# huzi96/gaussian-pcloud-render

Measured on AMD Instinct MI355X. Metric: rendered frames/sec at 1080p (fwd+bwd), THuman-800K, higher is better.
Workload: dtype f32

## Files before the change

### gaussian-pcloud-render_amd/csrc/api.hip

```cpp
#include <algorithm>
#include <cstdarg>
#include <cstdio>
#include <cstring>
#include <string>
#include <vector>

#include "common.hpp"
#include <atomic>
#include <map>
#include <mutex>

namespace gsr {

static thread_local char g_err[512] = "";

static int fail(int code, const char* fmt, ...)
{
    va_list ap;
    va_start(ap, fmt);
    vsnprintf(g_err, sizeof(g_err), fmt, ap);
    va_end(ap);
    return code;
}

// ... 117 lines not shown
        return fail(GSR_ERR_INVALID, "[gsr] %lld tiles x %d views: too many for one launch", (long long)(gx * gy), V);
    return GSR_OK;
}

static int tile_bits(int T) { return (int)higher_msb((uint32_t)T); }
static int sorted_buffer(int T) { return ((tile_bits(T) + RADIX_BITS - 1) / RADIX_BITS) & 1; }

static inline void* align256(void* p) { return (void*)(((uintptr_t)p + 255) & ~(uintptr_t)255); }

static int make_batch(const gsr_params* p, int V, void* geom, size_t geom_bytes, void* image, size_t image_bytes, void* binning,
                      size_t binning_bytes, bool with_grad, Batch& B)
{
    B.V = V;
    const size_t G = geom_view(nullptr, p->P).bytes, I = image_view(nullptr, p->W, p->H).bytes;
    const size_t GR = with_grad ? grad_rec_bytes(p->P) : 0;
    if (!geom || geom_bytes < (size_t)V * (G + GR) + 256)
        return fail(GSR_ERR_CAPACITY, "[gsr] geom arena too small (%zu < %zu%s)", geom_bytes, (size_t)V * (G + GR) + 256,
                    with_grad ? ", need_backward" : "");
    if (!image || image_bytes < (size_t)V * I + 256)
        return fail(GSR_ERR_CAPACITY, "[gsr] image arena too small (%zu < %zu)", image_bytes, (size_t)V * I + 256);
    B.g = geom_view(align256(geom), p->P);
    B.g_stride = G;
    B.grad_rec = with_grad ? reinterpret_cast<float*>(reinterpret_cast<char*>(align256(geom)) + (size_t)V * G) : nullptr;
    B.gr_stride = GR;
    B.iv = image_view(align256(image), p->W, p->H);
    B.iv_stride = I;
    if (binning) {
        if (binning_bytes < 256 + 256 * (size_t)V) return fail(GSR_ERR_CAPACITY, "[gsr] binning arena too small");
        const size_t per_view = ((binning_bytes - 256) / (size_t)V) / 256 * 256;
        const int64_t cap = bin_capacity_from_bytes(per_view);
        if (cap < 1) return fail(GSR_ERR_CAPACITY, "[gsr] binning arena too small (%zu bytes for %d views)", binning_bytes, V);
        B.b = bin_view(align256(binning), cap > 0xFFFFFFFFll ? 0xFFFFFFFFll : cap);
        B.b_stride = per_view;
    } else {
        B.b = bin_view(nullptr, 1);
        B.b.cap = 0;
        B.b_stride = 0;
    }
    return GSR_OK;
}

struct FrameRecord {
    int kind = 0;
    int need_backward = 0;
    int nx = 0, layout = 0;
    int V = 0, P = 0, W = 0, H = 0;
// ... 382 lines not shown
        int64_t n = list_pairs >= 0 ? list_pairs : B.b.cap;
        if (n > B.b.cap) n = B.b.cap;
        if (n < 1) n = 1;
        const size_t need = gsr_backward_det_bytes(V, p->P, p->W, p->H, n);
        if (!det->scratch || det->bytes < need)
            return fail(GSR_ERR_CAPACITY, "[gsr] backward_det: scratch block too small (%zu < %zu = gsr_backward_det_bytes(%d, %d, %d, %d, %lld): "
                        "the forward's lists hold up to %lld pairs per view)", det->bytes, need, V, p->P, p->W, p->H, (long long)n,
                        (long long)n);
        D = det_view(align256(det->scratch), T, n);
        d_stride = det_view_bytes(p->W, p->H, n);
    }
    if (x) {
        const int nx = x->X.nx;
        x->X.state = xstate_view(align256(const_cast<void*>(x->state)), p->W, p->H, B.b.cap, nx);
        x->X.state_stride = xstate_view_bytes(p->W, p->H, B.b.cap, nx);
        if (x->state_bytes < (size_t)V * x->X.state_stride + 256)
            return fail(GSR_ERR_CAPACITY, "[gsr] extra-state block too small for this binning arena");
    }
    {
        ProfScope ps("bwd_items", L.stream);
        const size_t n_out = !x ? 0 : (size_t)p->P * (x->layout == 0 ? x->X.nx : x->layout == 1 ? V * x->X.nx : (1 + V) * 4);
        if (x && hipMemsetAsync(x->XG.grad, 0, n_out * sizeof(float), L.stream) != hipSuccess)
            return fail(GSR_ERR_HIP, "[gsr] memset failed: %s", hipGetErrorString(hipGetLastError()));
        if (int e = launch_bwd_items(L, B, T, p->P)) return e;
    }
    int dres = 0;
    if (det) {
        {
            ProfScope ps("det_prepare", L.stream);
            if (int e = launch_det_prepare(L, B, D, d_stride, B.b.val[res], T)) return e;
        }
        {
            ProfScope ps("det_sort", L.stream);
            if (int e = launch_det_sort(L, B, D, d_stride, p->P, &dres)) return e;
        }
    }
    {
        ProfScope ps("render_backward", L.stream);
        const RenderBwdDet d{D.part, D.flags, D.slot_base, d_stride, (uint32_t)D.cap};
        if (int e = launch_render_backward(L, *p, B, B.b.val[res], G.dL_dpix, x ? &x->X : nullptr, x ? &x->XG : nullptr, det ? &d : nullptr))
            return e;
    }
    if (det) {
        ProfScope ps("det_reduce", L.stream);
        if (int e = launch_det_reduce(L, B, D, d_stride, dres)) return e;
    }
    {
// ... 279 lines not shown
```

### gaussian-pcloud-render_amd/csrc/binning.hip

```cpp
#include "common.hpp"
#include "tile_cull.hpp"

namespace gsr {

__device__ __forceinline__ uint64_t agent_load(const uint64_t* p)
{
    return __hip_atomic_load(p, __ATOMIC_RELAXED, __HIP_MEMORY_SCOPE_AGENT);
}
__device__ __forceinline__ void agent_store(uint64_t* p, uint64_t v)
{
    __hip_atomic_store(p, v, __ATOMIC_RELAXED, __HIP_MEMORY_SCOPE_AGENT);
}

#ifdef GSR_STATS
constexpr int DUP_REC = 65536;
__device__ unsigned g_dup_rec[DUP_REC][4];
#define DUP_T(var) const unsigned long long var = wall_clock64()
#define DUP_ADD(i, v) do { if (threadIdx.x == 0) { const unsigned r_ = blockIdx.y * gridDim.x + s_ticket; if (r_ < DUP_REC) g_dup_rec[r_][i] = (unsigned)(v); } } while (0)
int debug_dup_times(unsigned long long* out8, int reset)
{
    static unsigned host[DUP_REC][4];
    if (hipMemcpyFromSymbol(host, HIP_SYMBOL(g_dup_rec), sizeof(host)) != hipSuccess) return -1;
    for (int i = 0; i < 8; i++) out8[i] = 0;
    for (int r = 0; r < DUP_REC; r++) {
// ... 398 lines not shown
                cur[2 * lane + 1] = inc - a1;
            }
            __syncthreads();
        }
    }
}

static void order_params(float& knee, float& expo)
{
    static const float k = [] { const char* e = getenv("GSR_ORDER_KNEE"); return e ? (float)atof(e) : 2048.f; }();
    static const float x = [] { const char* e = getenv("GSR_ORDER_EXP"); return e ? (float)atof(e) : 0.3f; }();
    knee = k;
    expo = x;
}

int launch_tile_order(const Launch& L, const Batch& B, int T)
{
    float knee, expo;
    order_params(knee, expo);
    hipLaunchKernelGGL(k_tile_order, dim3(B.V), dim3(1024), 0, L.stream, T, B.iv.ranges, B.iv.tile_order, B.iv_stride, knee, expo);
    return check_launch(L, "tile_order");
}

constexpr int BWD_CLEAR_BLOCKS = 64;
__global__ __launch_bounds__(1024) void k_bwd_items(int T, int chunk_shift, const uint32_t* __restrict__ need, uint32_t* __restrict__ items,
                                                    uint32_t* __restrict__ count, size_t iv_stride, const uint64_t* __restrict__ counters,
                                                    size_t g_stride, float* __restrict__ grad_rec, size_t gr_stride, size_t gr_bytes)
{
    if (blockIdx.y != 0) {
        if (at_view(counters, g_stride, blockIdx.x)[CNT_BWD_DIRTY] == 0) return;
        zero_region(reinterpret_cast<char*>(at_view(grad_rec, gr_stride, blockIdx.x)), gr_bytes,
                    (size_t)(blockIdx.y - 1) * 1024 + threadIdx.x, (size_t)BWD_CLEAR_BLOCKS * 1024);
        return;
    }
    need = at_view(need, iv_stride, blockIdx.x);
    items = at_view(items, iv_stride, blockIdx.x);
    count = at_view(count, iv_stride, blockIdx.x);
    if (threadIdx.x < 8) count[BWD_QUEUE_WORD + threadIdx.x] = 0;
    __shared__ uint32_t cnt[ORD_BUCKETS];
    __shared__ uint32_t cur[ORD_BUCKETS];
    const uint32_t lane = threadIdx.x & 63;
    if (threadIdx.x < ORD_BUCKETS) cnt[threadIdx.x] = 0;
    __syncthreads();
    const uint32_t full_bucket = work_bucket(1u << chunk_shift);
    for (int pass = 0; pass < 2; pass++) {
        for (int t = threadIdx.x; t < T; t += 1024) {
            const uint32_t n = need[t];
            if (n == 0) continue;
            uint32_t n_full = n >> chunk_shift;
            if (n_full > BWD_MAX_CHUNKS - 1) n_full = BWD_MAX_CHUNKS - 1;
            const uint32_t rest = n - (n_full << chunk_shift);
            if (pass == 0) {
                if (n_full) atomicAdd(&cnt[full_bucket], n_full);
                if (rest) atomicAdd(&cnt[work_bucket(rest)], 1u);
            } else {
                if (n_full) {
                    const uint32_t slot = atomicAdd(&cur[full_bucket], n_full);
// ... 1 lines not shown
                }
                if (rest) items[atomicAdd(&cur[work_bucket(rest)], 1u)] = (uint32_t)t | (n_full << BWD_TILE_BITS);
            }
        }
        __syncthreads();
        if (pass == 0) {
            if (threadIdx.x < 64) {
                const uint32_t a0 = cnt[2 * lane], a1 = cnt[2 * lane + 1];
                uint32_t inc = a0 + a1;
#pragma unroll
                for (int d = 1; d < 64; d <<= 1) {
                    const uint32_t n = __shfl_up(inc, d, 64);
                    if (lane >= (uint32_t)d) inc += n;
                }
                cur[2 * lane] = inc - a0 - a1;
                cur[2 * lane + 1] = inc - a1;
                if (lane == 63) count[0] = inc;
            }
            __syncthreads();
        }
    }
}

int launch_bwd_items(const Launch& L, const Batch& B, int T, int P)
{
    hipLaunchKernelGGL(k_bwd_items, dim3(B.V, 1 + BWD_CLEAR_BLOCKS), dim3(1024), 0, L.stream, T, B.chunk_shift(), B.iv.tile_need, B.iv.bwd_items,
                       B.iv.bwd_count, B.iv_stride, B.g.counters, B.g_stride, B.grad_rec, B.gr_stride, grad_rec_bytes(P));
    return check_launch(L, "bwd_items");
}

}
```

### gaussian-pcloud-render_amd/csrc/common.hpp

```cpp
#pragma once
#include <hip/hip_runtime.h>
#include <stdint.h>

#include <type_traits>

#include "../../include/gsr.h"

#if defined(__HIP_DEVICE_COMPILE__) && !defined(__gfx950__)
#error "libgsr_hip is written for gfx950 (MI355X) only: build with --offload-arch=gfx950"
#endif

namespace gsr {

constexpr int TILE_X = 16;
constexpr int TILE_Y = 16;
constexpr int TILE_PIX = TILE_X * TILE_Y;

constexpr int RS_THREADS = 256;
constexpr int RS_WAVES = RS_THREADS / 64;
#ifndef GSR_RS_ITEMS
#define GSR_RS_ITEMS 16
#endif
constexpr int RS_ITEMS = GSR_RS_ITEMS;
constexpr int RS_TILE = RS_THREADS * RS_ITEMS;
// ... 10 lines not shown
#endif
constexpr int DUP_G = GSR_DUP_G;
constexpr int DUP_BLOCK = DUP_THREADS * DUP_G;
#ifndef GSR_DUP_COPIES
#define GSR_DUP_COPIES 8
#endif
constexpr int DUP_COPIES = GSR_DUP_COPIES;

inline size_t align_up(size_t v, size_t a) { return (v + a - 1) / a * a; }
inline int64_t div_up(int64_t a, int64_t b) { return (a + b - 1) / b; }

template <typename T>
__host__ __device__ __forceinline__ T* at_view(T* p, size_t stride_bytes, uint32_t view)
{
    using B = typename std::conditional<std::is_const<T>::value, const char, char>::type;
    return (T*)((B*)p + stride_bytes * view);
}

struct __attribute__((aligned(64))) Splat {
    float4 q0, q1, q2, q3;
};

constexpr int GRAD_REC_WORDS = 16;
inline size_t grad_rec_bytes(int P) { return ((size_t)(P > 0 ? P : 1) * GRAD_REC_WORDS * sizeof(float) + 255) / 256 * 256; }

constexpr int CNT_NUM_RENDERED = 0;
constexpr int CNT_TRAP = 1;
constexpr int CNT_STALL = 2;
constexpr int CNT_NUM_REFERENCE = 4;
constexpr int LAND_NUM_REFERENCE = 3;
constexpr int CNT_BWD_DIRTY = 3;

struct GeomView {
    Splat* splat;
    uint32_t* tiles_touched;
    uint8_t* clamped;
    uint32_t* dkey[2];
    uint32_t* dval[2];
    uint32_t* hist;
    uint32_t* totals;
    uint32_t* blk_minmax;
    uint32_t* sortctl;
    uint64_t* dup_status;
    uint64_t* counters;
    char* zero_begin;
    size_t zero_bytes;
    size_t bytes;
};

constexpr int BWD_CHUNK_SHIFT_MIN = 9;
#ifndef GSR_CHUNK_V
#define GSR_CHUNK_V 2
#endif
__host__ __device__ inline int bwd_chunk_shift(int V) { return V >= GSR_CHUNK_V ? 10 : 9; }
// ... 169 lines not shown
struct RenderBwdDet {
    float* part;
    uint32_t* flags;
    const uint32_t* slot_base;
    size_t stride;
    uint32_t cap;
};

struct Launch {
    hipStream_t stream;
    int debug;
};

struct Batch {
    int V;
    int chunk_shift() const { return bwd_chunk_shift(V); }
    GeomView g;
    size_t g_stride;
    ImageView iv;
    size_t iv_stride;
    BinView b;
    size_t b_stride;
    float* grad_rec;
    size_t gr_stride;
};

int check_launch(const Launch& L, const char* what);

int launch_preprocess(const Launch& L, const gsr_params& p, const Batch& B, int* radii);
int launch_recolor(const Launch& L, const gsr_params& p, const Batch& B, size_t colors_view_stride);
int launch_mark_visible(const Launch& L, int P, const float* means3D, const float* view, uint8_t* present);
struct SortJob {
    uint32_t* key[2];
    uint32_t* val[2];
    uint32_t* hist;
    uint32_t* totals;
    size_t stride;
    const uint64_t* n_dev;
    size_t n_stride;
    int64_t cap;
    int V;
    uint32_t* blk_minmax = nullptr;
    uint32_t* sortctl = nullptr;
    bool small_blocks = false;
};
constexpr int SORTCTL_BASE = 0;
constexpr int SORTCTL_BITS = 1;
constexpr uint32_t CULLED_KEY = 0xFFFFFFFFu;
__host__ __device__ inline uint32_t depth_sort_passes(uint32_t bits) { return (bits + RADIX_BITS - 1) / RADIX_BITS; }
int launch_radix_sort_pairs(const Launch& L, const SortJob& job, bool iota_vals, int end_bit, int* result_buffer, bool key16 = false);
int block_tickets(int set);
inline bool tile_keys16(int T) { return T <= 65536; }
int launch_duplicate(const Launch& L, int P, const Batch& B, int gridx, bool key16, uint64_t* host_land);
int launch_tile_ranges(const Launch& L, const Batch& B, const uint32_t* sorted_keys, int T, bool key16);
int launch_tile_order(const Launch& L, const Batch& B, int T);
int launch_bwd_items(const Launch& L, const Batch& B, int T, int P);
struct ExtraChannels {
    int nx;
    const float* values;
    const float* view_scale;
    const float* bg;
    float* out;
    size_t view_stride;
    const float* values_hi = nullptr;
    size_t hi_view_stride = 0;
    XStateView state{nullptr, nullptr, 0};
    size_t state_stride = 0;
};
struct ExtraGrads {
    const float* dL_dextra;
    float* grad;
    float* grad_hi;
};
int launch_render_forward(const Launch& L, const gsr_params& p, const Batch& B, const uint32_t* point_list, float* out_color,
                          bool with_ckpt, const ExtraChannels* X = nullptr);
int launch_render_backward(const Launch& L, const gsr_params& p, const Batch& B, const uint32_t* point_list, const float* dL_dpix,
                           const ExtraChannels* X = nullptr, const ExtraGrads* XG = nullptr, const RenderBwdDet* D = nullptr);
int backward_subquadrant_moments(int set);
int forward_half_views(int set);
// ... 27 lines not shown
```

### gaussian-pcloud-render_amd/csrc/preprocess.hip

```cpp
#include "common.hpp"
#include "splat_math.hpp"
#include "tile_cull.hpp"

namespace gsr {

template <int deg>
__device__ __forceinline__ V3 sh_to_rgb_t(V3 pos, V3 campos, const float* sh, uint32_t* clamp_mask)
{
    V3 dir = pos - campos;
    const float len = sqrtf(dot3(dir, dir));
    dir = v3(dir.x / len, dir.y / len, dir.z / len);
#define SHV(k) v3(sh[3 * (k)], sh[3 * (k) + 1], sh[3 * (k) + 2])
    V3 result = kSH_C0 * SHV(0);
    if constexpr (deg > 0) {
        const float x = dir.x, y = dir.y, z = dir.z;
        result = ((result - (kSH_C1 * y) * SHV(1)) + (kSH_C1 * z) * SHV(2)) - (kSH_C1 * x) * SHV(3);
        if constexpr (deg > 1) {
            const float xx = x * x, yy = y * y, zz = z * z;
            const float xy = x * y, yz = y * z, xz = x * z;
            result = result + (kSH_C2[0] * xy) * SHV(4);
            result = result + (kSH_C2[1] * yz) * SHV(5);
            result = result + (kSH_C2[2] * (2.0f * zz - xx - yy)) * SHV(6);
            result = result + (kSH_C2[3] * xz) * SHV(7);
            result = result + (kSH_C2[4] * (xx - yy)) * SHV(8);
// ... 26 lines not shown
    }
}

__device__ __forceinline__ float ndc_to_pix(float v, int S) { return (float)((((double)v + 1.0) * (double)S - 1.0) * 0.5); }

__device__ __forceinline__ uint32_t clamp_tile(float f, uint32_t grid)
{
    int v = (int)f;
    v = v > 0 ? v : 0;
    return grid < (uint32_t)v ? grid : (uint32_t)v;
}

struct PreArgs {
    int P, D, M, W, H, V, vpt;
    float tanfovx, tanfovy, focal_x, focal_y, scale_modifier;
    int prefiltered, need_backward, reference_lists;
    uint32_t gridx, gridy;
    const float *means3D, *shs, *colors_precomp, *opacities, *scales, *rotations, *cov3D_precomp;
    const float *view, *proj, *campos;
    Splat* splat;
    uint32_t* tiles_touched;
    uint8_t* clamped;
    uint32_t* dkey;
    float* grad_rec;
    uint64_t* counters;
    char* g_zero;
    size_t g_zero_bytes, g_stride, gr_stride;
    char* iv_zero;
    size_t iv_zero_bytes, iv_stride;
    int* radii;
};

template <int DEG>
__global__ __launch_bounds__(256) void k_preprocess(PreArgs a)
{
    const int v_first = blockIdx.y * a.vpt, v_last = v_first + a.vpt < a.V ? v_first + a.vpt : a.V;
    const int idx_raw = blockIdx.x * 256 + threadIdx.x;
    {
        const size_t gtid = (size_t)blockIdx.x * 256 + threadIdx.x, nthr = (size_t)gridDim.x * 256;
        for (int vw = v_first; vw < v_last; vw++) {
            if (gtid == 0) {
                at_view(a.counters, a.g_stride, vw)[CNT_STALL] = 0;
                at_view(a.counters, a.g_stride, vw)[CNT_BWD_DIRTY] = 0;
            }
            zero_region(a.g_zero + a.g_stride * vw, a.g_zero_bytes, gtid, nthr);
            zero_region(a.iv_zero + a.iv_stride * vw, a.iv_zero_bytes, gtid, nthr);
        }
    }
    const bool valid = idx_raw < a.P;
    const int idx = valid ? idx_raw : a.P - 1;
    __shared__ float4 xpose[4][256];

    const V3 p_orig = v3(a.means3D[3 * idx], a.means3D[3 * idx + 1], a.means3D[3 * idx + 2]);
    float cov6[6];
    if (a.cov3D_precomp) {
#pragma unroll
        for (int i = 0; i < 6; i++) cov6[i] = a.cov3D_precomp[6 * (size_t)idx + i];
    } else {
        const V3 sc = v3(a.scales[3 * idx], a.scales[3 * idx + 1], a.scales[3 * idx + 2]);
        const float4 q = *reinterpret_cast<const float4*>(a.rotations + 4 * (size_t)idx);
        cov3d_from_scale_rot(sc, a.scale_modifier, q, cov6, nullptr);
    }
    const float opacity = a.opacities[idx];
    V3 rgb_pre = v3(0, 0, 0);
    constexpr int NSH = 3 * (DEG + 1) * (DEG + 1);
    float shv[NSH];
    if (a.colors_precomp) {
// ... 86 lines not shown
                                                    __uint_as_float(tiles | SPANS_FLAG))
                                      : make_float4(__uint_as_float(rect.x), __uint_as_float(rect.y), __uint_as_float(etiles),
                                                    __uint_as_float(tiles));
        const int wave_first = idx_raw - (int)(threadIdx.x & 63);
        const bool full_wave = wave_first + 64 <= a.P;
        if (full_wave) {
            float4* mine = xpose[threadIdx.x >> 6] + 4 * (threadIdx.x & 63);
            mine[0] = s.q0; mine[1] = s.q1; mine[2] = s.q2; mine[3] = q3;
            __builtin_amdgcn_wave_barrier();
            const float4* rd = xpose[threadIdx.x >> 6] + (threadIdx.x & 63);
            float4* out = reinterpret_cast<float4*>(at_view(a.splat, a.g_stride, vw) + wave_first) + (threadIdx.x & 63);
            const float4 t0 = rd[0], t1 = rd[64], t2 = rd[128], t3 = rd[192];
            out[0] = t0; out[64] = t1; out[128] = t2; out[192] = t3;
            __builtin_amdgcn_wave_barrier();
        } else if (valid) {
            Splat* sp = at_view(a.splat, a.g_stride, vw) + idx;
            sp->q0 = s.q0;
            sp->q1 = s.q1;
            sp->q2 = s.q2;
            sp->q3 = q3;
        }
        if (a.need_backward && valid) {
            at_view(a.clamped, a.g_stride, vw)[idx] = (uint8_t)cmask;
            const float4 z = make_float4(0.f, 0.f, 0.f, 0.f);
            if (full_wave) {
                float4* recw = reinterpret_cast<float4*>(at_view(a.grad_rec, a.gr_stride, vw) + (size_t)wave_first * GRAD_REC_WORDS) + (threadIdx.x & 63);
                recw[0] = z; recw[64] = z; recw[128] = z; recw[192] = z;
            } else {
                float4* rec = reinterpret_cast<float4*>(at_view(a.grad_rec, a.gr_stride, vw) + (size_t)idx * GRAD_REC_WORDS);
                rec[0] = z; rec[1] = z; rec[2] = z; rec[3] = z;
            }
        }
    }
}

int launch_preprocess(const Launch& L, const gsr_params& p, const Batch& B, int* radii)
{
    const GeomView& g = B.g;
    PreArgs a;
    a.P = p.P; a.D = p.D; a.M = p.M; a.W = p.W; a.H = p.H;
    a.tanfovx = p.tanfovx; a.tanfovy = p.tanfovy;
    a.focal_y = p.H / (2.0f * p.tanfovy);
    a.focal_x = p.W / (2.0f * p.tanfovx);
    a.scale_modifier = p.scale_modifier;
    a.prefiltered = p.prefiltered;
    a.need_backward = p.need_backward;
    a.reference_lists = p.reference_lists;
    a.gridx = (uint32_t)((p.W + TILE_X - 1) / TILE_X);
    a.gridy = (uint32_t)((p.H + TILE_Y - 1) / TILE_Y);
    a.means3D = p.means3D; a.shs = p.shs; a.colors_precomp = p.colors_precomp; a.opacities = p.opacities;
    a.scales = p.scales; a.rotations = p.rotations; a.cov3D_precomp = p.cov3D_precomp;
    a.view = p.viewmatrix; a.proj = p.projmatrix; a.campos = p.campos;
    a.splat = g.splat; a.tiles_touched = g.tiles_touched; a.clamped = g.clamped;
    a.dkey = g.dkey[0]; a.radii = radii; a.counters = g.counters; a.grad_rec = B.grad_rec; a.gr_stride = B.gr_stride;
    a.g_zero = g.zero_begin; a.g_zero_bytes = g.zero_bytes; a.g_stride = B.g_stride;
    a.iv_zero = B.iv.zero_begin; a.iv_zero_bytes = B.iv.zero_bytes; a.iv_stride = B.iv_stride;
    const int blocks = (p.P + 255) / 256;
    a.V = B.V;
    a.vpt = 1;
    while (a.vpt < B.V && (int64_t)blocks * div_up(B.V, a.vpt * 2) >= 2048) a.vpt *= 2;
    if (a.vpt > B.V) a.vpt = B.V;
    const dim3 grid(blocks, (unsigned)div_up(B.V, a.vpt));
    switch (p.shs ? p.D : 0) {
    case 0: hipLaunchKernelGGL(k_preprocess<0>, grid, dim3(256), 0, L.stream, a); break;
    case 1: hipLaunchKernelGGL(k_preprocess<1>, grid, dim3(256), 0, L.stream, a); break;
    case 2: hipLaunchKernelGGL(k_preprocess<2>, grid, dim3(256), 0, L.stream, a); break;
    default: hipLaunchKernelGGL(k_preprocess<3>, grid, dim3(256), 0, L.stream, a); break;
    }
    return check_launch(L, "preprocess");
}

__global__ __launch_bounds__(256) void k_recolor(int P, int D, int M, const float* __restrict__ means3D,
                                                 const float* __restrict__ shs, const float* __restrict__ colors_precomp,
                                                 const float* __restrict__ campos, const uint32_t* __restrict__ tiles_touched,
                                                 Splat* __restrict__ splat, uint8_t* __restrict__ clamped, size_t g_stride,
                                                 size_t colors_view_stride)
{
// ... 48 lines not shown
```

### gaussian-pcloud-render_amd/csrc/preprocess_bwd.hip

```cpp
#include "common.hpp"
#include "splat_math.hpp"

namespace gsr {

__device__ __forceinline__ V3 dnormvdv(V3 v, V3 dv)
{
    const float sum2 = v.x * v.x + v.y * v.y + v.z * v.z;
    const float invsum32 = 1.0f / sqrtf(sum2 * sum2 * sum2);
    V3 r;
    r.x = ((+sum2 - v.x * v.x) * dv.x - v.y * v.x * dv.y - v.z * v.x * dv.z) * invsum32;
    r.y = (-v.x * v.y * dv.x + (sum2 - v.y * v.y) * dv.y - v.z * v.y * dv.z) * invsum32;
    r.z = (-v.x * v.z * dv.x - v.y * v.z * dv.y + (sum2 - v.z * v.z) * dv.z) * invsum32;
    return r;
}

template <int DEG> constexpr int sh_words() { return 3 * (DEG + 1) * (DEG + 1); }

struct PreBwdArgs {
    int P, D, M, V;
    int stage_sh;
    int stage_out;
    float tanfovx, tanfovy, focal_x, focal_y, scale_modifier;
    const float *means3D, *shs, *scales, *rotations, *cov3D_precomp;
    const float *view, *proj, *campos;
    const int* radii;
    const uint8_t* clamped;
    const float* grad_rec;
    size_t g_stride, gr_stride;
    uint64_t* counters;
    float *dL_dmean2D, *dL_dopacity, *dL_dcolor;
    float *dL_dmean3D, *dL_dcov3D, *dL_dsh, *dL_dscale, *dL_drot;
};

template <int deg>
__device__ __forceinline__ V3 sh_backward(V3 pos, V3 campos, const float* sh, uint32_t cmask, V3 dL_dRGB,
                                          float (&acc)[sh_words<deg>()])
{
    const V3 dir_orig = pos - campos;
    const float len = sqrtf(dot3(dir_orig, dir_orig));
    const V3 dir = v3(dir_orig.x / len, dir_orig.y / len, dir_orig.z / len);
    dL_dRGB.x *= (cmask & 1u) ? 0 : 1;
    dL_dRGB.y *= (cmask & 2u) ? 0 : 1;
    dL_dRGB.z *= (cmask & 4u) ? 0 : 1;
    V3 dRGBdx = v3(0, 0, 0), dRGBdy = v3(0, 0, 0), dRGBdz = v3(0, 0, 0);
    const float x = dir.x, y = dir.y, z = dir.z;
#define SHV(k) v3(sh[3 * (k)], sh[3 * (k) + 1], sh[3 * (k) + 2])
#define PUT(k, s) do { const V3 t_ = (s) * dL_dRGB; acc[3 * (k)] += t_.x; acc[3 * (k) + 1] += t_.y; acc[3 * (k) + 2] += t_.z; } while (0)
    PUT(0, kSH_C0);
    if constexpr (deg > 0) {
        PUT(1, -kSH_C1 * y);
        PUT(2, kSH_C1 * z);
        PUT(3, -kSH_C1 * x);
// ... 93 lines not shown
#pragma unroll
    for (int i = 0; i < NSH; i++) gsh[i] = 0.f;

    const V3 mean = v3(a.means3D[3 * idx], a.means3D[3 * idx + 1], a.means3D[3 * idx + 2]);
    float S6[6];
    V3 sc = v3(0, 0, 0);
    float4 q = make_float4(0, 0, 0, 0);
    if (a.cov3D_precomp) {
#pragma unroll
        for (int i = 0; i < 6; i++) S6[i] = a.cov3D_precomp[6 * (size_t)idx + i];
    } else {
        sc = v3(a.scales[3 * idx], a.scales[3 * idx + 1], a.scales[3 * idx + 2]);
        q = *reinterpret_cast<const float4*>(a.rotations + 4 * (size_t)idx);
        cov3d_from_scale_rot(sc, a.scale_modifier, q, S6, nullptr);
    }

    float shv[NSH];
    if (a.shs) {
        const float* shp = a.shs + (size_t)idx * a.M * 3;
#pragma unroll
        for (int i = 0; i < NSH; i++) shv[i] = shp[i];
    }

    for (int vw = 0; vw < a.V; vw++) {
        const float* recp = at_view(a.grad_rec, a.gr_stride, (uint32_t)vw) + (size_t)idx * GRAD_REC_WORDS;
        const float4 rec0 = *reinterpret_cast<const float4*>(recp);
        const float4 rec1 = *reinterpret_cast<const float4*>(recp + 4);
        const float rec8 = recp[8];
        g2x += rec0.x; g2y += rec0.y;
        gcol = gcol + v3(rec1.y, rec1.z, rec1.w);
        gop += rec8;
        if (!(a.radii[(size_t)vw * a.P + idx] > 0)) continue;

        const float* view = a.view + 16 * vw;
        const float* proj = a.proj + 16 * vw;
        const float fx = a.focal_x, fy = a.focal_y;
        const Cov2D c = cov2d_project(mean, fx, fy, a.tanfovx, a.tanfovy, S6, view);
        const bool clamp_x = c.txtz < -c.limx || c.txtz > c.limx, clamp_y = c.tytz < -c.limy || c.tytz > c.limy;
        const V3 m0 = v3(c.T.m[0][0], c.T.m[0][1], c.T.m[0][2]), m1 = v3(c.T.m[1][0], c.T.m[1][1], c.T.m[1][2]);
        const float ca = c.cov.m[0][0] + 0.3f, cb = c.cov.m[0][1], cc = c.cov.m[1][1] + 0.3f;

        const float gA = rec0.z, gB = rec0.w, gC = rec1.x;
        const float det = ca * cc - cb * cb;
        const float Dn = 1.0f / ((det * det) + 0.0000001f);
        float da = 0.f, db = 0.f, dc = 0.f;
        if (Dn != 0) {
            da = Dn * (-cc * cc * gA + 2 * cb * cc * gB + (det - ca * cc) * gC);
            dc = Dn * (-ca * ca * gC + 2 * ca * cb * gB + (det - ca * cc) * gA);
            db = Dn * 2 * (cb * cc * gA - (det + 2 * cb * cb) * gB + ca * cb * gC);
            gS[0] += m0.x * m0.x * da + m0.x * m1.x * db + m1.x * m1.x * dc;
            gS[3] += m0.y * m0.y * da + m0.y * m1.y * db + m1.y * m1.y * dc;
// ... 108 lines not shown
    for (int i = 0; i < 6; i++) a.dL_dcov3D[6 * (size_t)idx + i] = gS[i];

    if (a.scales) {
        a.dL_dscale[3 * (size_t)idx + 0] = dsc[0];
        a.dL_dscale[3 * (size_t)idx + 1] = dsc[1];
        a.dL_dscale[3 * (size_t)idx + 2] = dsc[2];
        *reinterpret_cast<float4*>(a.dL_drot + 4 * (size_t)idx) = dq;
    }
}

int launch_preprocess_backward(const Launch& L, const gsr_params& p, const Batch& B, const int* radii, float* dL_dmean2D,
                               float* dL_dopacity, float* dL_dcolor, float* dL_dmean3D, float* dL_dcov3D, float* dL_dsh,
                               float* dL_dscale, float* dL_drot)
{
    PreBwdArgs a;
    a.P = p.P; a.D = p.D; a.M = p.M; a.V = B.V;
    a.tanfovx = p.tanfovx; a.tanfovy = p.tanfovy;
    a.focal_y = p.H / (2.0f * p.tanfovy);
    a.focal_x = p.W / (2.0f * p.tanfovx);
    a.scale_modifier = p.scale_modifier;
    a.means3D = p.means3D; a.shs = p.shs; a.scales = p.scales; a.rotations = p.rotations;
    a.cov3D_precomp = p.cov3D_precomp; a.view = p.viewmatrix; a.proj = p.projmatrix; a.campos = p.campos;
    a.radii = radii; a.clamped = B.g.clamped;
    a.grad_rec = B.grad_rec; a.g_stride = B.g_stride; a.gr_stride = B.gr_stride; a.counters = B.g.counters;
    a.dL_dmean2D = dL_dmean2D; a.dL_dopacity = dL_dopacity; a.dL_dcolor = dL_dcolor;
    a.dL_dmean3D = dL_dmean3D; a.dL_dcov3D = dL_dcov3D; a.dL_dsh = dL_dsh; a.dL_dscale = dL_dscale; a.dL_drot = dL_drot;
    const dim3 grid((p.P + 255) / 256), block(256);
    size_t lds = p.shs ? (size_t)256 * 3 * p.M * sizeof(float) : 0;
    const auto al16 = [](const void* q) { return ((uintptr_t)q & 15u) == 0; };
    a.stage_sh = lds != 0 && lds <= 64 * 1024 && al16(dL_dsh);
    if (!a.stage_sh) lds = 0;
    const size_t lds_out = (size_t)(4 * 768 + 6 * 256) * sizeof(float);
    a.stage_out = al16(dL_dmean2D) && al16(dL_dcolor) && al16(dL_dmean3D) && al16(dL_dcov3D) && (!p.scales || al16(dL_dscale));
    if (a.stage_out && lds < lds_out) lds = lds_out;
    switch (p.shs ? p.D : 0) {
    case 0: hipLaunchKernelGGL(k_preprocess_backward<0>, grid, block, lds, L.stream, a); break;
    case 1: hipLaunchKernelGGL(k_preprocess_backward<1>, grid, block, lds, L.stream, a); break;
    case 2: hipLaunchKernelGGL(k_preprocess_backward<2>, grid, block, lds, L.stream, a); break;
    default: hipLaunchKernelGGL(k_preprocess_backward<3>, grid, block, lds, L.stream, a); break;
    }
    return check_launch(L, "preprocess_backward");
}

}
```

### gaussian-pcloud-render_amd/csrc/render_bwd.hip

```cpp
#include <atomic>
#include <cstdlib>

#include "common.hpp"
#include "tile_cull.hpp"

namespace gsr {

constexpr int BGRP = 4;
#ifndef GSR_BWD_SUBQ_DEFAULT
#define GSR_BWD_SUBQ_DEFAULT 2
#endif

#ifndef GSR_BWD_DIV
#define GSR_BWD_DIV 1
#endif
#ifndef GSR_BWD_NOFMA
#define GSR_BWD_NOFMA 0
#endif

typedef float f32x4 __attribute__((ext_vector_type(4)));

__device__ __forceinline__ void bw_prefetch16(f32x4& dst, const void* p)
{
    asm volatile("global_load_dwordx4 %0, %1, off" : "=v"(dst) : "v"(p) : "memory");
// ... 238 lines not shown
    out8[7] = (out8[7] << 20) | waves;
    if (reset) {
        for (int r = 0; r < BW_REC; r++) for (int i = 0; i < 8; i++) host[r][i] = 0;
        if (hipMemcpyToSymbol(HIP_SYMBOL(g_bwd_rec), host, sizeof(host)) != hipSuccess) return -1;
    }
    return 0;
}
#endif

struct RenderBwdArgs {
    const uint2* ranges;
    const uint32_t* items;
    const uint32_t* item_count;
    const float4* ckpt;
    const float* accum;
    const uint32_t* point_list;
    const Splat* splat;
    int W, H, gridx, num_tiles, chunk_shift;
    const float* bg;
    const float* final_T;
    const uint32_t* n_contrib;
    const float* dL_dpix;
    float* grad_rec;
    uint64_t* counters;
    uint32_t V;
    uint32_t dynamic;
    size_t g_stride, b_stride, iv_stride, gr_stride;
};

struct RenderBwdX {
    const float* extra;
    const float* extra_hi;
    size_t extra_vstride, extra_hi_vstride;
    const float* extra_scale;
    const float* bg_extra;
    const float4* xckpt;
    const float* xaccum;
    size_t x_stride;
    const float* dL_dextra;
    float* grad;
    float* grad_hi;
};

#ifndef GSR_SUBQ_M
#define GSR_SUBQ_M 20.f
#endif
constexpr float SUBQ_M = GSR_SUBQ_M;
// ... 23 lines not shown
    a.n_contrib = at_view(a.n_contrib, a.iv_stride, view);
    a.ckpt = at_view(a.ckpt, a.b_stride, view);
    a.point_list = at_view(a.point_list, a.b_stride, view);
    a.splat = at_view(a.splat, a.g_stride, view);
    a.grad_rec = at_view(a.grad_rec, a.gr_stride, view);
    a.dL_dpix += (size_t)view * 3u * (size_t)a.W * (size_t)a.H;
    const bool x_split = NX > 4 && x.extra_hi != nullptr;
    const uint32_t x_nx = x_split ? 4u : (uint32_t)NX;
    const float* const x_lo = NX > 0 ? x.extra + (size_t)view * x.extra_vstride : nullptr;
    const float* const x_hi = NX > 0 ? (x_split ? x.extra_hi + (size_t)view * x.extra_hi_vstride : x_lo + 4) : nullptr;
    float* const xg_lo = NX > 0 ? x.grad + (size_t)view * x.extra_vstride : nullptr;
    float* const xg_hi = NX > 0 ? (x_split ? x.grad_hi + (size_t)view * x.extra_hi_vstride : xg_lo + 4) : nullptr;
    float* det_part = nullptr;
    uint8_t* det_flag = nullptr;
    const uint32_t* det_base = nullptr;
    uint32_t det_pad = 0;
    if constexpr (DET) {
        det_part = at_view(det.part, det.stride, view);
        det_flag = reinterpret_cast<uint8_t*>(at_view(det.flags, det.stride, view));
        det_base = at_view(det.slot_base, det.stride, view);
        det_pad = (threadIdx.x >> 4) < 3u ? 9u + 2u * (threadIdx.x >> 4) + ((threadIdx.x >> 2) & 1u) : 15u;
    }
    const uint32_t n_items = at_view(a.item_count, a.iv_stride, view)[0];
    if (group < a.V && (blockIdx.x & 31u) == 0 && threadIdx.x == 0) at_view(a.counters, a.g_stride, view)[CNT_BWD_DIRTY] = 1;
    __shared__ __attribute__((aligned(16))) float stage[17 * QUAD_WORDS];
    __shared__ __attribute__((aligned(16))) float mrow[16 * MM_STRIDE];
    __shared__ __attribute__((aligned(16))) float stage_x[NX > 0 ? 16 * 4 * NX : 4];
#ifdef GSR_BWD_EMUL
    __shared__ float dpx_raster[3 * 64];
#endif
    float am[16];
    float amx[NX > 0 ? 16 : 1];
    mm_basis<SUBQ>(am, threadIdx.x);
    const uint32_t mm_p = mm_pos(threadIdx.x);
    const uint32_t mm_g = threadIdx.x >> 4, mm_j = threadIdx.x & 15u;
    const bool mm_u = mm_g == 3u && mm_j >= 8u;
    const uint32_t mm_gb = (mm_j >> 2) & 1u, mm_k4 = mm_j & 3u;
    const uint32_t mm_c2 = mm_g == 2u ? 8u : mm_g;
    const bool mm_onA = mm_g < 3u ? mm_j < 8u : (mm_j < 4u || mm_j >= 8u), mm_onB = mm_g < 3u ? mm_j < 8u : mm_j >= 4u;
    const uint32_t mm_cA = mm_g < 3u ? (mm_j < 4u ? 2u + mm_g : mm_c2) : (mm_j >= 12u ? 6u : mm_j >= 8u ? 5u : 7u);
    const uint32_t mm_cB = mm_g < 3u ? (mm_j < 4u ? mm_c2 : 2u + mm_g) : (mm_j >= 12u ? 5u : mm_j >= 8u ? 6u : 7u);
    const uint32_t mm_offP = mm_g == 0 ? 8u : 12u, mm_offQ = mm_g == 0 ? 12u : 16u;
    const float mm_dd = -(mm_g == 0 ? (float)(0.5 * a.W) : (float)(0.5 * a.H));
#ifdef GSR_STATS
    BW_T(tw0);
    unsigned long long tw_wait = 0, tw_setup = 0, tw_stage = 0, tw_eval = 0, n_rounds = 0, n_groups = 0, n_items_done = 0;
#endif
// ... 497 lines not shown
    }
    return v;
}

int launch_render_backward(const Launch& L, const gsr_params& p, const Batch& B, const uint32_t* point_list, const float* dL_dpix,
                           const ExtraChannels* X, const ExtraGrads* XG, const RenderBwdDet* D)
{
    RenderBwdArgs a;
    a.ranges = B.iv.ranges;
    a.items = B.iv.bwd_items;
    a.item_count = B.iv.bwd_count;
    a.ckpt = B.b.ckpt;
    a.accum = B.iv.accum;
    a.point_list = point_list;
    a.splat = B.g.splat;
    a.W = p.W; a.H = p.H;
    a.gridx = (p.W + TILE_X - 1) / TILE_X;
    const int gridy = (p.H + TILE_Y - 1) / TILE_Y;
    a.bg = p.bg;
    a.final_T = B.iv.final_T;
    a.n_contrib = B.iv.n_contrib;
    a.dL_dpix = dL_dpix;
    a.grad_rec = B.grad_rec; a.gr_stride = B.gr_stride;
    a.counters = B.g.counters;
    a.num_tiles = a.gridx * gridy;
    a.chunk_shift = B.chunk_shift();
    a.V = (uint32_t)B.V;
    a.g_stride = B.g_stride; a.b_stride = B.b_stride; a.iv_stride = B.iv_stride;
    static const int cus = [] { int dev = 0, n = 0; (void)hipGetDevice(&dev); (void)hipDeviceGetAttribute(&n, hipDeviceAttributeMultiprocessorCount, dev); return n > 0 ? n : 256; }();
    int64_t groups = div_up(a.num_tiles, 8);
#ifndef GSR_BWD_FILL
#define GSR_BWD_FILL 4096
#endif
    a.dynamic = (B.V > 1 && groups * B.V > GSR_BWD_FILL) ? 1u : 0u;
    if (a.dynamic) groups = div_up((int64_t)cus * 4 * 5 * 2, 32 * (int64_t)B.V);
    if (groups < 8) groups = 8;
    const dim3 grid((unsigned)(groups * B.V) * 32u);
    if (X != nullptr && X->nx > 0) {
        RenderBwdX x;
        x.extra = X->values; x.extra_hi = X->values_hi; x.extra_vstride = X->view_stride; x.extra_hi_vstride = X->hi_view_stride;
        x.extra_scale = X->view_scale; x.bg_extra = X->bg;
        x.xckpt = X->state.ckpt; x.xaccum = X->state.accum; x.x_stride = X->state_stride;
        x.dL_dextra = XG->dL_dextra; x.grad = XG->grad; x.grad_hi = XG->grad_hi;
        const int mode = backward_subquadrant_moments(-1);
#define GSR_LAUNCH_BWD_X(M_, NX_) hipLaunchKernelGGL((k_render_backward<M_, NX_, RenderBwdX>), grid, dim3(64), 0, L.stream, a, x)
        if (X->nx == 4) {
            if (mode == 1) GSR_LAUNCH_BWD_X(1, 4); else if (mode == 2) GSR_LAUNCH_BWD_X(2, 4); else GSR_LAUNCH_BWD_X(0, 4);
// ... 25 lines not shown
```

### gaussian-pcloud-render_amd/diff_gaussian_rasterization/_native.py

```python
import ctypes as C
import os
import threading
import weakref as _weakref

import torch

_HERE = os.path.dirname(os.path.abspath(__file__))
LIB_PATH = os.environ.get("GSR_LIB") or os.path.join(_HERE, "libgsr_hip.so")

_fp = C.c_void_p


class GsrParams(C.Structure):
    _fields_ = [
        ("P", C.c_int), ("D", C.c_int), ("M", C.c_int), ("W", C.c_int), ("H", C.c_int),
        ("tanfovx", C.c_float), ("tanfovy", C.c_float), ("scale_modifier", C.c_float),
        ("prefiltered", C.c_int), ("debug", C.c_int), ("need_backward", C.c_int), ("reference_lists", C.c_int),
        ("bg", _fp), ("means3D", _fp), ("shs", _fp), ("colors_precomp", _fp), ("opacities", _fp),
        ("scales", _fp), ("rotations", _fp), ("cov3D_precomp", _fp),
        ("viewmatrix", _fp), ("projmatrix", _fp), ("campos", _fp),
    ]


GSR_RETRY = 1
# ... 677 lines not shown

def query(name, P, W, H, R, geom, binning, img, view=0, n_views=1):
    if name in ("POINT_LIST", "POINT_LIST_KEYS"):
        R = int(query("LIST_PAIRS", P, W, H, R, geom, binning, img, view=view, n_views=n_views)[0])
    dtype, shp = _QSPEC[name]
    T = ((W + 15) // 16) * ((H + 15) // 16)
    out = torch.zeros(shp(P, R, T, W * H), dtype=dtype, device=geom.device)
    if out.numel() == 0:
        return out
    p = GsrParams()
    p.P, p.W, p.H = P, W, H
    g_stride, i_stride = lib.gsr_geom_bytes_inference(P) - 256, lib.gsr_image_bytes(W, H) - 256
    b_stride = ((binning.numel() - 256) // n_views) // 256 * 256 if binning.numel() else 0
    if geom.data_ptr() % 256 or img.data_ptr() % 256 or (binning.numel() and binning.data_ptr() % 256):
        raise RuntimeError("query: arena base pointers are expected to be 256-byte aligned")
    with torch.cuda.device(geom.device):
        _check(lib.gsr_query(C.byref(p), Q[name], geom.data_ptr() + view * g_stride,
                             (binning.data_ptr() + view * b_stride) if binning.numel() else None, b_stride + 256,
                             img.data_ptr() + view * i_stride, int(R), out.data_ptr(), out.numel() * out.element_size(),
                             _stream_handle(geom.device)))
    return out


def grad_records(geom, P, view=0, n_views=1):
    g_stride = lib.gsr_geom_bytes_inference(P) - 256
    gr_stride = lib.gsr_geom_bytes(P) - lib.gsr_geom_bytes_inference(P)
    if geom.data_ptr() % 256:
        raise RuntimeError("grad_records: arena base pointers are expected to be 256-byte aligned")
    if geom.numel() < n_views * (g_stride + gr_stride):
        raise RuntimeError("grad_records: not a need_backward geometry arena of %d views" % n_views)
    off = n_views * g_stride + view * gr_stride
    return geom[off:off + P * 64].view(torch.float32).view(P, 16).clone()


class ClockProbe:

    def __init__(self, device, capacity=256, iters=256):
        self.device, self.iters, self.n, self._mu = device, int(iters), 0, threading.Lock()
        with torch.cuda.device(device):
            self.buf = torch.zeros((capacity, 2), dtype=torch.int64, device=device)
            self.stream = torch.cuda.Stream(device=device)
            self.khz = int(lib.gsr_wall_clock_khz())
        torch.cuda.synchronize(device)

    def launch(self):
        with self._mu:
            if self.n >= self.buf.shape[0]:
                return
            slot = self.n
            self.n += 1
        with torch.cuda.device(self.device):
            _check(lib.gsr_clock_probe_launch(self.buf.data_ptr() + 16 * slot, self.iters, self.stream.cuda_stream))

    def mhz(self, first=0):
        self.stream.synchronize()
# ... 25 lines not shown
```

Measured before the change: 2123.

## Zero only touched gradient records via per-point live flags instead of full clears

```diff
diff --git a/gaussian-pcloud-render_amd/csrc/api.hip b/gaussian-pcloud-render_amd/csrc/api.hip
--- a/gaussian-pcloud-render_amd/csrc/api.hip
+++ b/gaussian-pcloud-render_amd/csrc/api.hip
@@ -163,6 +163,7 @@
     B.g = geom_view(align256(geom), p->P);
     B.g_stride = G;
     B.grad_rec = with_grad ? reinterpret_cast<float*>(reinterpret_cast<char*>(align256(geom)) + (size_t)V * G) : nullptr;
+    B.grad_flag = with_grad ? reinterpret_cast<uint8_t*>(B.grad_rec) + grad_flag_offset(p->P) : nullptr;
     B.gr_stride = GR;
     B.iv = image_view(align256(image), p->W, p->H);
     B.iv_stride = I;
@@ -591,7 +592,11 @@
         const size_t n_out = !x ? 0 : (size_t)p->P * (x->layout == 0 ? x->X.nx : x->layout == 1 ? V * x->X.nx : (1 + V) * 4);
         if (x && hipMemsetAsync(x->XG.grad, 0, n_out * sizeof(float), L.stream) != hipSuccess)
             return fail(GSR_ERR_HIP, "[gsr] memset failed: %s", hipGetErrorString(hipGetLastError()));
-        if (int e = launch_bwd_items(L, B, T, p->P)) return e;
+        if (int e = launch_bwd_items(L, B, T)) return e;
+    }
+    {
+        ProfScope ps("bwd_mark_clear", L.stream);
+        if (int e = launch_bwd_mark_clear(L, B, B.b.val[res], T, p->P)) return e;
     }
     int dres = 0;
     if (det) {
diff --git a/gaussian-pcloud-render_amd/csrc/binning.hip b/gaussian-pcloud-render_amd/csrc/binning.hip
--- a/gaussian-pcloud-render_amd/csrc/binning.hip
+++ b/gaussian-pcloud-render_amd/csrc/binning.hip
@@ -444,17 +444,9 @@
     return check_launch(L, "tile_order");
 }
 
-constexpr int BWD_CLEAR_BLOCKS = 64;
 __global__ __launch_bounds__(1024) void k_bwd_items(int T, int chunk_shift, const uint32_t* __restrict__ need, uint32_t* __restrict__ items,
-                                                    uint32_t* __restrict__ count, size_t iv_stride, const uint64_t* __restrict__ counters,
-                                                    size_t g_stride, float* __restrict__ grad_rec, size_t gr_stride, size_t gr_bytes)
-{
-    if (blockIdx.y != 0) {
-        if (at_view(counters, g_stride, blockIdx.x)[CNT_BWD_DIRTY] == 0) return;
-        zero_region(reinterpret_cast<char*>(at_view(grad_rec, gr_stride, blockIdx.x)), gr_bytes,
-                    (size_t)(blockIdx.y - 1) * 1024 + threadIdx.x, (size_t)BWD_CLEAR_BLOCKS * 1024);
-        return;
-    }
+                                                    uint32_t* __restrict__ count, size_t iv_stride)
+{
     need = at_view(need, iv_stride, blockIdx.x);
     items = at_view(items, iv_stride, blockIdx.x);
     count = at_view(count, iv_stride, blockIdx.x);
@@ -502,11 +494,70 @@
     }
 }
 
-int launch_bwd_items(const Launch& L, const Batch& B, int T, int P)
-{
-    hipLaunchKernelGGL(k_bwd_items, dim3(B.V, 1 + BWD_CLEAR_BLOCKS), dim3(1024), 0, L.stream, T, B.chunk_shift(), B.iv.tile_need, B.iv.bwd_items,
-                       B.iv.bwd_count, B.iv_stride, B.g.counters, B.g_stride, B.grad_rec, B.gr_stride, grad_rec_bytes(P));
+int launch_bwd_items(const Launch& L, const Batch& B, int T)
+{
+    hipLaunchKernelGGL(k_bwd_items, dim3(B.V), dim3(1024), 0, L.stream, T, B.chunk_shift(), B.iv.tile_need, B.iv.bwd_items,
+                       B.iv.bwd_count, B.iv_stride);
     return check_launch(L, "bwd_items");
 }
 
-}
+__global__ __launch_bounds__(256) void k_bwd_mark(int P, int chunk_shift, const uint32_t* __restrict__ need, const uint2* __restrict__ ranges,
+                                                   const uint32_t* __restrict__ items, const uint32_t* __restrict__ count,
+                                                   size_t iv_stride, const uint32_t* __restrict__ point_list, size_t b_stride,
+                                                   uint8_t* __restrict__ flag, size_t gr_stride)
+{
+    const uint32_t view = blockIdx.y, lane = threadIdx.x & 63u;
+    need = at_view(need, iv_stride, view);
+    ranges = at_view(ranges, iv_stride, view);
+    items = at_view(items, iv_stride, view);
+    point_list = at_view(point_list, b_stride, view);
+    flag = at_view(flag, gr_stride, view);
+    const uint32_t n_items = at_view(count, iv_stride, view)[0];
+    for (uint32_t it = blockIdx.x * 4u + (threadIdx.x >> 6); it < n_items; it += gridDim.x * 4u) {
+        const uint32_t item = items[it];
+        const uint32_t tile = item & ((1u << BWD_TILE_BITS) - 1u), chunk = item >> BWD_TILE_BITS;
+        const uint32_t total = need[tile], lo = chunk << chunk_shift;
+        if (lo >= total) continue;
+        const bool last_chunk = chunk == BWD_MAX_CHUNKS - 1 || lo + (1u << chunk_shift) >= total;
+        const uint32_t hi = last_chunk ? total : lo + (1u << chunk_shift);
+        const uint32_t* plist = point_list + ranges[tile].x;
+#pragma unroll 4
+        for (uint32_t i = lo + lane; i < hi; i += 64u) {
+            const uint32_t id = plist[i];
+            if (id < (uint32_t)P) flag[id] = 1;
+        }
+    }
+}
+
+__global__ __launch_bounds__(256) void k_bwd_clear(int P, const uint8_t* __restrict__ flag, float* __restrict__ grad_rec, size_t gr_stride)
+{
+    const uint32_t view = blockIdx.y, lane = threadIdx.x & 63u;
+    const uint32_t idx = blockIdx.x * 256u + threadIdx.x;
+    const uint32_t wave_first = idx - lane;
+    if (wave_first >= (uint32_t)P) return;
+    const bool on = idx < (uint32_t)P && at_view(flag, gr_stride, view)[idx] != 0;
+    const uint64_t mask = __ballot(on);
+    float4* rec = reinterpret_cast<float4*>(at_view(grad_rec, gr_stride, view) + (size_t)wave_first * GRAD_REC_WORDS);
+#pragma unroll
+    for (uint32_t g = 0; g < 4u; g++) {
+        const uint32_t k = g * 16u + (lane >> 2);
+        if ((mask >> k) & 1ull) rec[g * 64u + lane] = make_float4(0.f, 0.f, 0.f, 0.f);
+    }
+}
+
+int launch_bwd_mark_clear(const Launch& L, const Batch& B, const uint32_t* point_list, int T, int P)
+{
+    int64_t items = (int64_t)T + (B.b.cap >> B.chunk_shift());
+    if (items > (int64_t)BWD_MAX_CHUNKS * T) items = (int64_t)BWD_MAX_CHUNKS * T;
+    int64_t blocks = div_up(items, 4);
+    blocks = blocks < 1 ? 1 : blocks > 4096 ? 4096 : blocks;
+    hipLaunchKernelGGL(k_bwd_mark, dim3((unsigned)blocks, B.V), dim3(256), 0, L.stream, P, B.chunk_shift(), (const uint32_t*)B.iv.tile_need,
+                       (const uint2*)B.iv.ranges, (const uint32_t*)B.iv.bwd_items, (const uint32_t*)B.iv.bwd_count, B.iv_stride, point_list,
+                       B.b_stride, B.grad_flag, B.gr_stride);
+    if (int e = check_launch(L, "bwd_mark")) return e;
+    hipLaunchKernelGGL(k_bwd_clear, dim3((unsigned)div_up(P, 256), B.V), dim3(256), 0, L.stream, P, (const uint8_t*)B.grad_flag, B.grad_rec,
+                       B.gr_stride);
+    return check_launch(L, "bwd_clear");
+}
+
+}
diff --git a/gaussian-pcloud-render_amd/csrc/common.hpp b/gaussian-pcloud-render_amd/csrc/common.hpp
--- a/gaussian-pcloud-render_amd/csrc/common.hpp
+++ b/gaussian-pcloud-render_amd/csrc/common.hpp
@@ -56,14 +56,14 @@
 };
 
 constexpr int GRAD_REC_WORDS = 16;
-inline size_t grad_rec_bytes(int P) { return ((size_t)(P > 0 ? P : 1) * GRAD_REC_WORDS * sizeof(float) + 255) / 256 * 256; }
+inline size_t grad_flag_offset(int P) { return (size_t)(P > 0 ? P : 1) * GRAD_REC_WORDS * sizeof(float); }
+inline size_t grad_rec_bytes(int P) { return align_up(grad_flag_offset(P) + (size_t)(P > 0 ? P : 1), 256); }
 
 constexpr int CNT_NUM_RENDERED = 0;
 constexpr int CNT_TRAP = 1;
 constexpr int CNT_STALL = 2;
 constexpr int CNT_NUM_REFERENCE = 4;
 constexpr int LAND_NUM_REFERENCE = 3;
-constexpr int CNT_BWD_DIRTY = 3;
 
 struct GeomView {
     Splat* splat;
@@ -279,6 +279,7 @@
     BinView b;
     size_t b_stride;
     float* grad_rec;
+    uint8_t* grad_flag;
     size_t gr_stride;
 };
 
@@ -311,7 +312,8 @@
 int launch_duplicate(const Launch& L, int P, const Batch& B, int gridx, bool key16, uint64_t* host_land);
 int launch_tile_ranges(const Launch& L, const Batch& B, const uint32_t* sorted_keys, int T, bool key16);
 int launch_tile_order(const Launch& L, const Batch& B, int T);
-int launch_bwd_items(const Launch& L, const Batch& B, int T, int P);
+int launch_bwd_items(const Launch& L, const Batch& B, int T);
+int launch_bwd_mark_clear(const Launch& L, const Batch& B, const uint32_t* point_list, int T, int P);
 struct ExtraChannels {
     int nx;
     const float* values;
diff --git a/gaussian-pcloud-render_amd/csrc/preprocess.hip b/gaussian-pcloud-render_amd/csrc/preprocess.hip
--- a/gaussian-pcloud-render_amd/csrc/preprocess.hip
+++ b/gaussian-pcloud-render_amd/csrc/preprocess.hip
@@ -72,7 +72,7 @@
     uint32_t* tiles_touched;
     uint8_t* clamped;
     uint32_t* dkey;
-    float* grad_rec;
+    uint8_t* grad_flag;
     uint64_t* counters;
     char* g_zero;
     size_t g_zero_bytes, g_stride, gr_stride;
@@ -89,10 +89,7 @@
     {
         const size_t gtid = (size_t)blockIdx.x * 256 + threadIdx.x, nthr = (size_t)gridDim.x * 256;
         for (int vw = v_first; vw < v_last; vw++) {
-            if (gtid == 0) {
-                at_view(a.counters, a.g_stride, vw)[CNT_STALL] = 0;
-                at_view(a.counters, a.g_stride, vw)[CNT_BWD_DIRTY] = 0;
-            }
+            if (gtid == 0) at_view(a.counters, a.g_stride, vw)[CNT_STALL] = 0;
             zero_region(a.g_zero + a.g_stride * vw, a.g_zero_bytes, gtid, nthr);
             zero_region(a.iv_zero + a.iv_stride * vw, a.iv_zero_bytes, gtid, nthr);
         }
@@ -225,14 +222,7 @@
         }
         if (a.need_backward && valid) {
             at_view(a.clamped, a.g_stride, vw)[idx] = (uint8_t)cmask;
-            const float4 z = make_float4(0.f, 0.f, 0.f, 0.f);
-            if (full_wave) {
-                float4* recw = reinterpret_cast<float4*>(at_view(a.grad_rec, a.gr_stride, vw) + (size_t)wave_first * GRAD_REC_WORDS) + (threadIdx.x & 63);
-                recw[0] = z; recw[64] = z; recw[128] = z; recw[192] = z;
-            } else {
-                float4* rec = reinterpret_cast<float4*>(at_view(a.grad_rec, a.gr_stride, vw) + (size_t)idx * GRAD_REC_WORDS);
-                rec[0] = z; rec[1] = z; rec[2] = z; rec[3] = z;
-            }
+            at_view(a.grad_flag, a.gr_stride, vw)[idx] = 0;
         }
     }
 }
@@ -255,7 +245,7 @@
     a.scales = p.scales; a.rotations = p.rotations; a.cov3D_precomp = p.cov3D_precomp;
     a.view = p.viewmatrix; a.proj = p.projmatrix; a.campos = p.campos;
     a.splat = g.splat; a.tiles_touched = g.tiles_touched; a.clamped = g.clamped;
-    a.dkey = g.dkey[0]; a.radii = radii; a.counters = g.counters; a.grad_rec = B.grad_rec; a.gr_stride = B.gr_stride;
+    a.dkey = g.dkey[0]; a.radii = radii; a.counters = g.counters; a.grad_flag = B.grad_flag; a.gr_stride = B.gr_stride;
     a.g_zero = g.zero_begin; a.g_zero_bytes = g.zero_bytes; a.g_stride = B.g_stride;
     a.iv_zero = B.iv.zero_begin; a.iv_zero_bytes = B.iv.zero_bytes; a.iv_stride = B.iv_stride;
     const int blocks = (p.P + 255) / 256;
diff --git a/gaussian-pcloud-render_amd/csrc/preprocess_bwd.hip b/gaussian-pcloud-render_amd/csrc/preprocess_bwd.hip
--- a/gaussian-pcloud-render_amd/csrc/preprocess_bwd.hip
+++ b/gaussian-pcloud-render_amd/csrc/preprocess_bwd.hip
@@ -26,8 +26,8 @@
     const int* radii;
     const uint8_t* clamped;
     const float* grad_rec;
+    const uint8_t* grad_flag;
     size_t g_stride, gr_stride;
-    uint64_t* counters;
     float *dL_dmean2D, *dL_dopacity, *dL_dcolor;
     float *dL_dmean3D, *dL_dcov3D, *dL_dsh, *dL_dscale, *dL_drot;
 };
@@ -167,11 +167,18 @@
         for (int i = 0; i < NSH; i++) shv[i] = shp[i];
     }
 
+    uint32_t live_next = a.grad_flag[idx];
     for (int vw = 0; vw < a.V; vw++) {
-        const float* recp = at_view(a.grad_rec, a.gr_stride, (uint32_t)vw) + (size_t)idx * GRAD_REC_WORDS;
-        const float4 rec0 = *reinterpret_cast<const float4*>(recp);
-        const float4 rec1 = *reinterpret_cast<const float4*>(recp + 4);
-        const float rec8 = recp[8];
+        const uint32_t live = live_next;
+        if (vw + 1 < a.V) live_next = at_view(a.grad_flag, a.gr_stride, (uint32_t)vw + 1u)[idx];
+        float4 rec0 = make_float4(0.f, 0.f, 0.f, 0.f), rec1 = rec0;
+        float rec8 = 0.f;
+        if (live) {
+            const float* recp = at_view(a.grad_rec, a.gr_stride, (uint32_t)vw) + (size_t)idx * GRAD_REC_WORDS;
+            rec0 = *reinterpret_cast<const float4*>(recp);
+            rec1 = *reinterpret_cast<const float4*>(recp + 4);
+            rec8 = recp[8];
+        }
         g2x += rec0.x; g2y += rec0.y;
         gcol = gcol + v3(rec1.y, rec1.z, rec1.w);
         gop += rec8;
@@ -326,7 +333,7 @@
     a.means3D = p.means3D; a.shs = p.shs; a.scales = p.scales; a.rotations = p.rotations;
     a.cov3D_precomp = p.cov3D_precomp; a.view = p.viewmatrix; a.proj = p.projmatrix; a.campos = p.campos;
     a.radii = radii; a.clamped = B.g.clamped;
-    a.grad_rec = B.grad_rec; a.g_stride = B.g_stride; a.gr_stride = B.gr_stride; a.counters = B.g.counters;
+    a.grad_rec = B.grad_rec; a.grad_flag = B.grad_flag; a.g_stride = B.g_stride; a.gr_stride = B.gr_stride;
     a.dL_dmean2D = dL_dmean2D; a.dL_dopacity = dL_dopacity; a.dL_dcolor = dL_dcolor;
     a.dL_dmean3D = dL_dmean3D; a.dL_dcov3D = dL_dcov3D; a.dL_dsh = dL_dsh; a.dL_dscale = dL_dscale; a.dL_drot = dL_drot;
     const dim3 grid((p.P + 255) / 256), block(256);
diff --git a/gaussian-pcloud-render_amd/csrc/render_bwd.hip b/gaussian-pcloud-render_amd/csrc/render_bwd.hip
--- a/gaussian-pcloud-render_amd/csrc/render_bwd.hip
+++ b/gaussian-pcloud-render_amd/csrc/render_bwd.hip
@@ -284,7 +284,6 @@
     const uint32_t* n_contrib;
     const float* dL_dpix;
     float* grad_rec;
-    uint64_t* counters;
     uint32_t V;
     uint32_t dynamic;
     size_t g_stride, b_stride, iv_stride, gr_stride;
@@ -354,7 +353,6 @@
         det_pad = (threadIdx.x >> 4) < 3u ? 9u + 2u * (threadIdx.x >> 4) + ((threadIdx.x >> 2) & 1u) : 15u;
     }
     const uint32_t n_items = at_view(a.item_count, a.iv_stride, view)[0];
-    if (group < a.V && (blockIdx.x & 31u) == 0 && threadIdx.x == 0) at_view(a.counters, a.g_stride, view)[CNT_BWD_DIRTY] = 1;
     __shared__ __attribute__((aligned(16))) float stage[17 * QUAD_WORDS];
     __shared__ __attribute__((aligned(16))) float mrow[16 * MM_STRIDE];
     __shared__ __attribute__((aligned(16))) float stage_x[NX > 0 ? 16 * 4 * NX : 4];
@@ -898,7 +896,6 @@
     a.n_contrib = B.iv.n_contrib;
     a.dL_dpix = dL_dpix;
     a.grad_rec = B.grad_rec; a.gr_stride = B.gr_stride;
-    a.counters = B.g.counters;
     a.num_tiles = a.gridx * gridy;
     a.chunk_shift = B.chunk_shift();
     a.V = (uint32_t)B.V;
diff --git a/gaussian-pcloud-render_amd/diff_gaussian_rasterization/_native.py b/gaussian-pcloud-render_amd/diff_gaussian_rasterization/_native.py
--- a/gaussian-pcloud-render_amd/diff_gaussian_rasterization/_native.py
+++ b/gaussian-pcloud-render_amd/diff_gaussian_rasterization/_native.py
@@ -723,15 +723,26 @@
     return out
 
 
-def grad_records(geom, P, view=0, n_views=1):
+def _grad_block(geom, P, view, n_views):
     g_stride = lib.gsr_geom_bytes_inference(P) - 256
     gr_stride = lib.gsr_geom_bytes(P) - lib.gsr_geom_bytes_inference(P)
     if geom.data_ptr() % 256:
         raise RuntimeError("grad_records: arena base pointers are expected to be 256-byte aligned")
     if geom.numel() < n_views * (g_stride + gr_stride):
         raise RuntimeError("grad_records: not a need_backward geometry arena of %d views" % n_views)
-    off = n_views * g_stride + view * gr_stride
-    return geom[off:off + P * 64].view(torch.float32).view(P, 16).clone()
+    return n_views * g_stride + view * gr_stride, max(P, 1) * 64
+
+
+def grad_record_flags(geom, P, view=0, n_views=1):
+    off, flags = _grad_block(geom, P, view, n_views)
+    return geom[off + flags:off + flags + P].clone()
+
+
+def grad_records(geom, P, view=0, n_views=1):
+    off, flags = _grad_block(geom, P, view, n_views)
+    rec = geom[off:off + P * 64].view(torch.float32).view(P, 16)
+    live = geom[off + flags:off + flags + P] != 0
+    return torch.where(live[:, None], rec, torch.zeros_like(rec))
 
 
 class ClockProbe:
```

After: 2055. 3.2% lower.
